# NVlabs/sionna

Measured on NVIDIA H100. Metric: coded bits/s, LDPC5G n=8448 k=4224 BP-20 decode, higher is better.
Workload: dtype f32

## Files before the change

include/sionna_b200.h:

```cpp
#ifndef SIONNA_B200_H
#define SIONNA_B200_H
#include <stddef.h>
#include <stdint.h>

#ifdef __cplusplus
extern "C" {
#endif

#define SB_OK 0
#define SB_EINVAL (-1)
#define SB_ECUDA (-2)
#define SB_ENOMEM (-3)
#define SB_EUNSUPPORTED (-4)

const char* sb_last_error(void);
int sb_device_info(int* sm_count, int* cc_major, int* cc_minor, int* smem_optin_bytes);
int sb_version(void);
int64_t sb_launch_count(void);

typedef struct sb_ldpc_graph sb_ldpc_graph;

enum { SB_CN_BOXPLUS_PHI = 0, SB_CN_BOXPLUS = 1, SB_CN_MINSUM = 2, SB_CN_OFFSET_MINSUM = 3, SB_CN_IDENTITY = 4 };
enum { SB_VN_SUM = 0, SB_VN_IDENTITY = 1 };

int sb_ldpc_graph_create(sb_ldpc_graph** out, int32_t num_cn, int32_t num_vn, int32_t num_edges,
                         const int32_t* h_cn_of_edge, const int32_t* h_vn_of_edge,
                         const int32_t* h_in_map, int32_t n_in,
                         const int32_t* h_out_vn, int32_t n_out,
                         const int32_t* h_schedule, int32_t n_sub, int32_t n_active);
int sb_ldpc_graph_create_ordered(sb_ldpc_graph** out, int32_t num_cn, int32_t num_vn, int32_t num_edges,
                                 const int32_t* h_cn_of_edge, const int32_t* h_vn_of_edge,
                                 const int32_t* h_in_map, int32_t n_in,
                                 const int32_t* h_out_vn, int32_t n_out,
                                 const int32_t* h_schedule, int32_t n_sub, int32_t n_active,
                                 const int32_t* h_cn_view);
void sb_ldpc_graph_destroy(sb_ldpc_graph* g);
int sb_ldpc_graph_set_qc(sb_ldpc_graph* g, int32_t Z, int32_t n_entries, const int32_t* h_base_row,
                         const int32_t* h_base_col, const int32_t* h_shift);
int sb_ldpc_graph_is_qc(const sb_ldpc_graph* g);
int sb_debug_phi(const float* d_x, float* d_scalar, float* d_packed, int64_t n, void* stream);
int sb_ldpc_graph_on_chip(const sb_ldpc_graph* g);
size_t sb_ldpc_workspace_bytes(const sb_ldpc_graph* g);
int sb_ldpc_graph_export(const sb_ldpc_graph* g, int32_t* dims, int32_t* cn_order, int32_t* vn_order,
                         int32_t* slot_of_edge, int32_t* vn_slot, int32_t* cn_off, int32_t* vn_off);

int sb_ldpc_decode(const sb_ldpc_graph* g, const float* d_llr, int64_t batch, int32_t num_iter,
                   int32_t cn_rule, int32_t vn_rule, float offset, float llr_max, int32_t hard_out,
                   const float* d_state_in, float* d_state_out, float* d_out,
                   void* d_workspace, size_t workspace_bytes, void* stream);

int sb_ldpc_decode_early(const sb_ldpc_graph* g, const float* d_llr, int64_t batch, int32_t max_iter, int32_t cn_rule,
                         float offset, float llr_max, int32_t hard_out, float* d_out, int32_t* d_num_iter, void* stream);

int sb_ldpc_flat_init(const float* d_x, const int32_t* d_vn_of_edge, const float* d_state_in, float* d_llr, float* d_v2c,
                      int64_t batch, int32_t num_vn, int32_t num_edges, void* stream);
int sb_ldpc_flat_cn(const float* d_v2c, float* d_c2v, const int32_t* d_cn_ptr, const int32_t* d_v2c_perm,
                    const int32_t* d_cn_list, int32_t num_nodes, int64_t batch, int32_t cn_rule, float offset,
                    float llr_max, void* stream);
int sb_ldpc_flat_vn(const float* d_c2v, const float* d_llr, const int32_t* d_vn_ptr, const int32_t* d_c2v_perm,
                    float* d_v2c, float* d_xhat, int32_t num_vn, int64_t batch, int32_t vn_rule, float llr_max,
                    void* stream);
int sb_ldpc_flat_out(const float* d_xhat, const int32_t* d_out_vn, float* d_out, const float* d_v2c, float* d_state_out,
                     int64_t batch, int32_t n_out, int32_t num_edges, int32_t hard_out, void* stream);

typedef struct sb_ldpc5g_encoder sb_ldpc5g_encoder;
int sb_ldpc5g_encoder_create(sb_ldpc5g_encoder** out, int32_t k, int32_t n, int32_t k_ldpc, int32_t n_ldpc,
                             int32_t g_rows, const int32_t* h_a_ptr, const int32_t* h_a_idx,
                             const int32_t* h_binv_ptr, const int32_t* h_binv_idx, const int32_t* h_c1_ptr,
                             const int32_t* h_c1_idx, const int32_t* h_c2_ptr, const int32_t* h_c2_idx,
                             const int32_t* h_tx_vn);
void sb_ldpc5g_encoder_destroy(sb_ldpc5g_encoder* e);
int sb_ldpc5g_encode(const sb_ldpc5g_encoder* e, const float* d_u, int64_t batch, float* d_c, void* stream);

int sb_binary_source(float* d_out, int64_t n, uint64_t seed, uint64_t offset, void* stream);
int sb_normal(float* d_out, int64_t n, float mean, float stddev, uint64_t seed, uint64_t offset, void* stream);
int sb_uniform(float* d_out, int64_t n, float lo, float hi, uint64_t seed, uint64_t offset, void* stream);
int sb_qam_map(const float* d_bits, const float* d_points, int32_t m, float* d_out, int32_t* d_idx_out,
               int64_t n_sym, void* stream);
int sb_demap(const float* d_y, const float* d_no, int64_t no_inner, const float* d_points, int32_t m, int32_t method,
             const float* d_prior, int64_t prior_inner, float* d_llr, int64_t n_sym, int32_t hard_out, void* stream);
int sb_demap_qam(const float* d_y, const float* d_no, int64_t no_inner, const float* d_levels_re,
                 const float* d_levels_im, int32_t m, int32_t method, float* d_llr, int64_t n_sym, int32_t hard_out,
                 void* stream);
int sb_symbol_demap(const float* d_y, const float* d_no, int64_t no_inner, const float* d_points, int32_t num_points,
                    const float* d_prior, int64_t prior_inner, void* d_out, int64_t n_sym, int32_t hard_out,
                    void* stream);
int sb_awgn(const float* d_x, const float* d_no, int64_t no_inner, float* d_y, int64_t n, uint64_t seed,
            uint64_t offset, void* stream);
int sb_count_errors(const float* d_b, const float* d_b_hat, int64_t rows, int32_t k, int64_t* d_counters, void* stream);

int sb_crc_encode(const float* d_bits, const uint32_t* d_gen_rows, int32_t k, int32_t crc_length, float* d_out,
                  int64_t rows, void* stream);
// ... 170 lines not shown
```

sionna_b200/_lib.py:

```python
import ctypes as C
import os

_HERE = os.path.dirname(os.path.abspath(__file__))
LIB_PATH = os.environ.get("SIONNA_B200_LIB") or os.path.join(_HERE, "libsionna_b200.so")
_lib = None

i32, i64, u64, f32, vp, sz = C.c_int32, C.c_int64, C.c_uint64, C.c_float, C.c_void_p, C.c_size_t
P_i32 = C.POINTER(C.c_int32)

SIGNATURES = {
    "sb_last_error": (C.c_char_p, []),
    "sb_device_info": (i32, [P_i32, P_i32, P_i32, P_i32]),
    "sb_version": (i32, []),
    "sb_launch_count": (i64, []),
    "sb_ldpc_graph_create": (i32, [C.POINTER(vp), i32, i32, i32, vp, vp, vp, i32, vp, i32, vp, i32, i32]),
    "sb_ldpc_graph_create_ordered": (i32, [C.POINTER(vp), i32, i32, i32, vp, vp, vp, i32, vp, i32, vp, i32, i32, vp]),
    "sb_ldpc_graph_destroy": (None, [vp]),
    "sb_ldpc_graph_set_qc": (i32, [vp, i32, i32, vp, vp, vp]),
    "sb_ldpc_graph_is_qc": (i32, [vp]),
    "sb_debug_phi": (i32, [vp, vp, vp, i64, vp]),
    "sb_ldpc_graph_on_chip": (i32, [vp]),
    "sb_ldpc_workspace_bytes": (sz, [vp]),
    "sb_ldpc_decode": (i32, [vp, vp, i64, i32, i32, i32, f32, f32, i32, vp, vp, vp, vp, sz, vp]),
    "sb_ldpc_decode_early": (i32, [vp, vp, i64, i32, i32, f32, f32, i32, vp, vp, vp]),
    "sb_ldpc_flat_init": (i32, [vp, vp, vp, vp, vp, i64, i32, i32, vp]),
    "sb_ldpc_flat_cn": (i32, [vp, vp, vp, vp, vp, i32, i64, i32, f32, f32, vp]),
    "sb_ldpc_flat_vn": (i32, [vp, vp, vp, vp, vp, vp, i32, i64, i32, f32, vp]),
    "sb_ldpc_flat_out": (i32, [vp, vp, vp, vp, vp, i64, i32, i32, i32, vp]),
    "sb_ldpc_graph_export": (i32, [vp, vp, vp, vp, vp, vp, vp, vp]),
    "sb_ldpc5g_encoder_create": (i32, [C.POINTER(vp), i32, i32, i32, i32, i32] + [vp] * 9),
    "sb_ldpc5g_encoder_destroy": (None, [vp]),
    "sb_ldpc5g_encode": (i32, [vp, vp, i64, vp, vp]),
    "sb_binary_source": (i32, [vp, i64, u64, u64, vp]),
    "sb_normal": (i32, [vp, i64, f32, f32, u64, u64, vp]),
    "sb_qam_map": (i32, [vp, vp, i32, vp, vp, i64, vp]),
    "sb_demap": (i32, [vp, vp, i64, vp, i32, i32, vp, i64, vp, i64, i32, vp]),
    "sb_demap_qam": (i32, [vp, vp, i64, vp, vp, i32, i32, vp, i64, i32, vp]),
    "sb_symbol_demap": (i32, [vp, vp, i64, vp, i32, vp, i64, vp, i64, i32, vp]),
    "sb_awgn": (i32, [vp, vp, i64, vp, i64, u64, u64, vp]),
    "sb_count_errors": (i32, [vp, vp, i64, i32, vp, vp]),
    "sb_crc_encode": (i32, [vp, vp, i32, i32, vp, i64, vp]),
    "sb_crc_check": (i32, [vp, vp, i32, i32, vp, vp, i64, vp]),
    "sb_scramble": (i32, [vp, vp, i32, vp, i64, i32, i32, vp]),
    "sb_ofdm_modulate": (i32, [vp, vp, i64, i32, i32, vp, vp, i32, i32, vp]),
    "sb_ofdm_demodulate": (i32, [vp, vp, i64, i32, i32, vp, vp, i32, i32, i32, vp]),
    "sb_gather_rows": (i32, [vp, vp, vp, i64, i32, i32, i32, i32, i32, vp]),
    "sb_rg_map": (i32, [vp, vp, vp, vp, i64, i32, i32, i32, i32, vp]),
    "sb_ls_at_pilots": (i32, [vp, vp, vp, vp, i64, vp, vp, i64, i32, i32, i32, vp]),
    "sb_interp_lin": (i32, [vp] * 8 + [i32, vp, i64, i32, i32, i32, i32, i32, vp]),
    "sb_apply_ofdm_channel": (i32, [vp, vp, vp, i64, vp, i64, i32, i32, i32, i32, u64, u64, vp]),
    "sb_apply_time_channel": (i32, [vp, vp, vp, i64, vp, i64, i32, i32, i32, i32, i32, u64, u64, vp]),
    "sb_uniform": (i32, [vp, i64, f32, f32, u64, u64, vp]),
    "sb_tdl_sos": (i32, [vp, vp, vp, vp, vp, f32, f32, vp, i64, i32, i32, i32, i32, f32, vp]),
    "sb_cdl_coefficients": (i32, [vp] * 15 + [f32, f32, vp, i64, i32, i32, i32, i32, f32, vp]),
    "sb_phase_table": (i32, [vp, vp, f32, i32, vp, i64, i32, i32, vp]),
    "sb_cir_gram": (i32, [vp, vp, i64, i32, i32, vp]),
    "sb_cir_link_scale": (i32, [vp, vp, i64, vp, i64, i32, i32, i32, i32, i32, i32, f32, vp]),
    "sb_cir_apply": (i32, [vp, vp, i64, vp, vp, i64, i32, i32, i32, i32, i32, i32, i32, vp]),
    "sb_spatial_corr": (i32, [vp, vp, vp, i64, i32, i64, vp]),
    "sb_flat_fading": (i32, [vp, i64, u64, u64, vp, i64, vp, i64, i32, vp, vp, i64, vp, i64, u64, u64, vp, i64, i32, i32, vp]),
    "sb_chol_lower": (i32, [vp, vp, i64, i32, vp]),
    "sb_pusch_precode": (i32, [vp, vp, vp, i64, i32, i32, i32, i64, vp]),
    "sb_pusch_ls_combine": (i32, [vp, vp, i64, i32, i32, i32, i32, vp]),
    "sb_lmmse_equalize": (i32, [vp, vp, vp, vp, vp, i64, i32, i32, vp]),
    "sb_mimo_linalg": (i32, [i32, vp, vp, vp, vp, vp, i64, i32, i32, vp]),
    "sb_ofdm_frontend": (i32, [vp] * 15 + [i64] + [i32] * 11 + [vp]),
    "sb_ofdm_lmmse": (i32, [vp] * 12 + [i64] + [i32] * 8 + [vp]),
    "sb_ofdm_equalize": (i32, [i32] + [vp] * 12 + [i64] + [i32] * 8 + [vp]),
    "sb_mimo_ml": (i32, [vp] * 7 + [sz, i64] + [i32] * 6 + [vp]),
    "sb_ml_workspace_bytes": (sz, [i64, i32]),
    "sb_ofdm_ml": (i32, [vp] * 14 + [sz, i64] + [i32] * 12 + [vp]),
    "sb_mimo_kbest": (i32, [vp] * 6 + [sz, i64] + [i32] * 7 + [f32, vp]),
# ... 89 lines not shown
```

sionna_b200/csrc/ldpc_bp_qc.cu:

```cuda
#include <algorithm>
#include <climits>
#include <iterator>
#include <numeric>
#include <vector>
#include "sb_common.h"
#include "sb_math.h"
#include "sb_math2.cuh"
#include "ldpc_graph.h"
#include "ldpc_rules.cuh"

namespace {

constexpr int kLoop = INT_MAX;
constexpr int kRowMax[] = {kLoop, 20, 12, 8, 4};
constexpr int kColCut = 7, kColFused = 10;
constexpr int kColMax[] = {kLoop, 32, 20, 12, 8, 4, 2, kLoop, 12, 4, 1};
constexpr int kRowClasses = (int)std::size(kRowMax);
constexpr int kColClasses = (int)std::size(kColMax);

constexpr bool decreasing(const int* m, int lo, int hi) {
    for (int k = lo + 1; k < hi; ++k)
        if (m[k] >= m[k - 1]) return false;
    return true;
}
static_assert(decreasing(kRowMax, 0, kRowClasses), "row class bounds must decrease");
static_assert(decreasing(kColMax, 0, kColCut) && decreasing(kColMax, kColCut, kColFused), "column class bounds must decrease");
static_assert(kColFused == kColClasses - 1 && kColMax[kColFused] == 1, "the fused class holds degree-1 columns only");

constexpr int degree_class(const int* m, int lo, int hi, int d) {
    int k = hi - 1;
    while (k > lo && d > m[k]) --k;
    return k;
}

struct QcParams {
    int Z, n_rows, n_cols, nnz, N, E, E_alloc, n_in, n_out;
    int row_cls_end[kRowClasses];
    int col_cls_end[kColClasses];
    int row_cls_mod[kRowClasses];
    int col_cls_mod[kColClasses];
    const int4* row_info;
    const int4* col_info;
    const int2* col_edge;
    const int* in_idx;
    const int* out_pos;
    const int* slot_of_edge;
    const float* llr;
    float* out;
    float* state_out;
    long long B;
    int num_iter, hard_out, use_tma;
    int early;
    int* iters_out;
    const int2* row_edge;
    int tab_rep;
    float offset, llr_max;
};


#define SB_PHI_HI 16.635532f
#define SB_PHI_ZERO 14.7117348f
template <class LT, class Probe>
__device__ __forceinline__ uint2 phi_pass1_pair(unsigned b0, unsigned b1, float& P, const LT& lt, Probe probe) {
    const float a0 = __uint_as_float(b0 & 0x7fffffffu), a1 = __uint_as_float(b1 & 0x7fffffffu);
    const float2 p = sb_phif2(make_float2(a0, a1), lt);
    probe(a0, a1);
    P = __fadd_rn(P, p.x);
    P = __fadd_rn(P, p.y);
    return make_uint2(__float_as_uint(p.x) | (b0 & 0x80000000u), __float_as_uint(p.y) | (b1 & 0x80000000u));
}
template <class LT>
__device__ __forceinline__ unsigned phi_pass1(unsigned b0, float& P, const LT& lt) {
    const float p = sb_phif_s(__uint_as_float(b0 & 0x7fffffffu), lt);
    P = __fadd_rn(P, p);
    return __float_as_uint(p) | (b0 & 0x80000000u);
}
template <class LT>
__device__ __forceinline__ uint2 phi_pass2_pair(unsigned w0, unsigned w1, float P, unsigned par, float clip, const LT& lt) {
    const float2 m = fadd2(make_float2(__uint_as_float(w0 | 0x80000000u), __uint_as_float(w1 | 0x80000000u)),
                           make_float2(P, P));
    const float2 y = sb_phif2(m, lt);
    return make_uint2(__float_as_uint(fminf(y.x, clip)) | ((w0 ^ par) & 0x80000000u),
                      __float_as_uint(fminf(y.y, clip)) | ((w1 ^ par) & 0x80000000u));
}
template <class LT>
__device__ __forceinline__ unsigned phi_pass2(unsigned w0, float P, unsigned par, float clip, const LT& lt) {
    const float y = sb_phif_s(__fadd_rn(__uint_as_float(w0 | 0x80000000u), P), lt);
    return __float_as_uint(fminf(y, clip)) | ((w0 ^ par) & 0x80000000u);
}
__device__ __forceinline__ unsigned ldw(const float* q) { return __float_as_uint(*q); }
__device__ __forceinline__ void stw(float* q, unsigned w) { *q = __uint_as_float(w); }

template <class LT>
__device__ __noinline__ void cn_phi_qc(float* pm, int Z, int deg, float clip, int* sat_flag, LT lt) {
    const unsigned am = __activemask();
    float P = 0.f;
    unsigned par = 0;
    int l = 0;
#pragma unroll 2
    for (; l + 1 < deg; l += 2) {
        float* q0 = pm + l * Z;
        float* q1 = q0 + Z;
        const unsigned b0 = ldw(q0), b1 = ldw(q1);
        par ^= b0 ^ b1;
        const uint2 w = phi_pass1_pair(b0, b1, P, lt, [&](float a0, float a1) {
            if (l == 0 && __all_sync(am, a0 >= SB_PHI_HI && a1 >= SB_PHI_HI)) *sat_flag = 1;
        });
        stw(q0, w.x);
        stw(q1, w.y);
// ... 206 lines not shown
    uint32_t j4, j4w, jk;
};
__device__ __forceinline__ uint32_t vn_addr(int2 e, const VnLane& v) {
    return (uint32_t)e.x + (v.jk < (uint32_t)e.y ? v.j4w : v.j4);
}
__device__ __forceinline__ bool vn_in_row(int2 e, uint32_t addr, const VnLane& v) {
    return addr - (uint32_t)e.x - ((uint32_t)e.y >> 16) < ((uint32_t)e.y & 0xffffu);
}

template <int DMAX, bool CHECK, bool KEEPM, bool EXACT = false>
__device__ __forceinline__ float vn_qc(uint32_t ce_s, int deg, const VnLane& vl, float llr, float clip) {
    uint32_t addr[DMAX];
    float m[KEEPM ? DMAX : 1];
    bool on[DMAX];
    float acc = 0.f;
#pragma unroll
    for (int k = 0; k < DMAX; ++k) {
        int2 e = make_int2(0, 0);
        if (EXACT || k < deg) e = lds_i2(ce_s + 8 * k);
        addr[k] = vn_addr(e, vl);
        bool ok = EXACT || ((k < deg) && (!CHECK || vn_in_row(e, addr[k], vl)));
        on[k] = ok;
        float v = 0.f;
        if (ok) v = lds_f32(addr[k]);
        if (ok) acc = __fadd_rn(acc, v);
        if (KEEPM) m[KEEPM ? k : 0] = v;
    }
    float x_tot = __fadd_rn(acc, llr);
#pragma unroll
    for (int k = 0; k < DMAX; ++k) {
        float v = 0.f;
        if (KEEPM) v = m[KEEPM ? k : 0];
        else if (on[k]) v = lds_f32(addr[k]);
        float y = clipf(__fadd_rn(-v, x_tot), clip);
        if (on[k]) sts_f32(addr[k], y);
    }
    return x_tot;
}

template <int MODE>
__device__ __forceinline__ float vn_qc_loop(uint32_t ce_s, int deg, const VnLane& vl, float llr, float clip) {
    float acc = 0.f;
    if (MODE == 0)
        for (int k = 0; k < deg; ++k) {
            const int2 e = lds_i2(ce_s + 8 * k);
            const uint32_t a = vn_addr(e, vl);
            if (vn_in_row(e, a, vl)) acc = __fadd_rn(acc, lds_f32(a));
        }
    float x_tot = __fadd_rn(acc, llr);
    for (int k = 0; k < deg; ++k) {
        const int2 e = lds_i2(ce_s + 8 * k);
        const uint32_t a = vn_addr(e, vl);
        if (vn_in_row(e, a, vl))
            sts_f32(a, (MODE == 1) ? __fadd_rn(llr, 0.f) : clipf(__fadd_rn(-lds_f32(a), x_tot), clip));
    }
    return x_tot;
}

template <int CLS, bool EX>
__device__ __forceinline__ float vn_cls(uint32_t ce, int deg, const VnLane& vl, float llr, float clip) {
    constexpr int D = kColMax[CLS];
    if constexpr (D == kLoop) {
        return vn_qc_loop<0>(ce, deg, vl, llr, clip);
    } else if constexpr (CLS >= kColCut) {
        return vn_qc<D, true, true>(ce, deg, vl, llr, clip);
    } else if constexpr (D > 12) {
        if (CLS == 2 && EX && deg == 19) return vn_qc<19, false, true, true>(ce, deg, vl, llr, clip);
        if (CLS == 2 && EX && deg == 17) return vn_qc<17, false, true, true>(ce, deg, vl, llr, clip);
        return vn_qc<D, false, false>(ce, deg, vl, llr, clip);
    } else {
        if constexpr (CLS == 3) {
            if (EX && deg == 9) return vn_qc<9, false, true, true>(ce, deg, vl, llr, clip);
            if (EX && deg == 10) return vn_qc<10, false, true, true>(ce, deg, vl, llr, clip);
            if (EX && deg == 11) return vn_qc<11, false, true, true>(ce, deg, vl, llr, clip);
        } else if constexpr (CLS == 4) {
            if (EX && deg == 5) return vn_qc<5, false, true, true>(ce, deg, vl, llr, clip);
            if (EX && deg == 6) return vn_qc<6, false, true, true>(ce, deg, vl, llr, clip);
            if (EX && deg == 7) return vn_qc<7, false, true, true>(ce, deg, vl, llr, clip);
        } else if constexpr (CLS == 5) {
            if (EX && deg == 3) return vn_qc<3, false, true, true>(ce, deg, vl, llr, clip);
        } else {
            if (EX && deg == 1) return vn_qc<1, false, true, true>(ce, deg, vl, llr, clip);
        }
        return vn_qc<D, false, true, EX>(ce, deg, vl, llr, clip);
    }
}

struct WarpCtx {
    int G, grp, lane_i;
};

__device__ __forceinline__ int first_of(int start, int start_mod, const WarpCtx& w) {
    return start + (w.grp - start_mod + (w.grp < start_mod ? w.G : 0));
}

__device__ __forceinline__ void fused_vn(const QcParams& p, float* q, float c2v, int fw, int lane_i, const float* llr_s,
                                         float clip, unsigned char* hd) {
    int s = fw >> 16, vb = fw & 0xffff;
    int j = lane_i + s;
    j -= (j >= p.Z) ? p.Z : 0;
    float x_tot = __fadd_rn(__fadd_rn(0.f, c2v), llr_s[vb * p.Z + j]);
    *q = clipf(__fadd_rn(-c2v, x_tot), clip);
    if (hd) hd[vb * p.Z + j] = 0.f >= x_tot ? 1 : 0;
}

template <int RULE, int CLS, class LT>
__device__ __forceinline__ void cn_class(const QcParams& p, const WarpCtx& w, float* msg, const float* llr_s,
// ... 104 lines not shown
        const int4 ri = s_row[rr];
        if (w.lane_i < ri.z) {
            unsigned par = 0;
            for (int l = 0; l < ri.y; ++l) {
                const int2 e = __ldg(p.row_edge + ri.x + l);
                int j = w.lane_i + e.y;
                j -= (j >= p.Z) ? p.Z : 0;
                par ^= hd[e.x + j];
            }
            if (par) *unsat = 1;
        }
    }
}

template <int CLS, bool EX>
__device__ __forceinline__ void vn_class(const QcParams& p, const WarpCtx& w, const VnLane& vl, const float* llr_s,
                                         const int4* s_col, uint32_t s_ce, int start, int end, float clip,
                                         bool final_pass, long long b, unsigned char* hd) {
    for (int cc = first_of(start, p.col_cls_mod[CLS], w); cc < end; cc += w.G) {
        int4 ci = s_col[cc];
        if (w.lane_i < ci.z) {
            int v = ci.w + w.lane_i;
            float x_tot = vn_cls<CLS, EX>(s_ce + 8 * ci.x, ci.y, vl, llr_s[v], clip);
            if (hd) hd[v] = 0.f >= x_tot ? 1 : 0;
            if (final_pass) {
                int o = p.out_pos[v];
                if (o >= 0) {
                    x_tot = clipf(x_tot, clip);
                    p.out[(size_t)b * p.n_out + o] = decoder_out(x_tot, p.hard_out);
                }
            }
        }
    }
}

template <bool EX>
__device__ __forceinline__ void vn_all(const QcParams& p, const WarpCtx& w, const VnLane& vl, const float* llr_s,
                                       const int4* s_col, uint32_t s_ce, float clip, bool final_pass,
                                       bool with_fused, long long b, unsigned char* hd) {
    const int* ce = p.col_cls_end;
    vn_class<0, EX>(p, w, vl, llr_s, s_col, s_ce, 0, ce[0], clip, final_pass, b, hd);
    vn_class<1, EX>(p, w, vl, llr_s, s_col, s_ce, ce[0], ce[1], clip, final_pass, b, hd);
    vn_class<2, EX>(p, w, vl, llr_s, s_col, s_ce, ce[1], ce[2], clip, final_pass, b, hd);
    vn_class<3, EX>(p, w, vl, llr_s, s_col, s_ce, ce[2], ce[3], clip, final_pass, b, hd);
    vn_class<4, EX>(p, w, vl, llr_s, s_col, s_ce, ce[3], ce[4], clip, final_pass, b, hd);
    vn_class<5, EX>(p, w, vl, llr_s, s_col, s_ce, ce[4], ce[5], clip, final_pass, b, hd);
    vn_class<6, EX>(p, w, vl, llr_s, s_col, s_ce, ce[5], ce[6], clip, final_pass, b, hd);
    vn_class<7, EX>(p, w, vl, llr_s, s_col, s_ce, ce[6], ce[7], clip, final_pass, b, hd);
    vn_class<8, EX>(p, w, vl, llr_s, s_col, s_ce, ce[7], ce[8], clip, final_pass, b, hd);
    vn_class<9, EX>(p, w, vl, llr_s, s_col, s_ce, ce[8], ce[9], clip, final_pass, b, hd);
    if (with_fused) vn_class<10, EX>(p, w, vl, llr_s, s_col, s_ce, ce[9], ce[10], clip, final_pass, b, hd);
}

__device__ __forceinline__ void vn_init(const QcParams& p, const WarpCtx& w, const VnLane& vl, const float* llr_s,
                                        const int4* s_col, uint32_t s_ce) {
    for (int cc = w.grp; cc < p.n_cols; cc += w.G) {
        const int4 ci = s_col[cc];
        if (w.lane_i < ci.z) vn_qc_loop<1>(s_ce + 8 * ci.x, ci.y, vl, llr_s[ci.w + w.lane_i], 0.f);
    }
}

constexpr int kQcThreads = 768;

template <int RULE, int REP, bool EARLY>
__global__ void __launch_bounds__(kQcThreads, 1) ldpc_bp_qc_kernel(const __grid_constant__ QcParams p) {
    const int T = blockDim.x, tid = threadIdx.x, lane = tid & 31, warp = tid >> 5, W = T >> 5;
    const int Z = p.Z, N = p.N, Zb = (Z + 31) >> 5;
    unsigned char* const smem_raw = sb_smem + (RULE == SB_CN_BOXPLUS_PHI ? LogTab<REP>::bytes : 0);
    const int off_llr = p.E_alloc * 4;
    const int off_col = (off_llr + N * 4 + 15) & ~15;
    const int off_row = off_col + p.n_cols * 16;
    const int off_ce = off_row + p.n_rows * 16;
    const int off_bar = (off_ce + p.nnz * 8 + 15) & ~15;
    float* msg = reinterpret_cast<float*>(smem_raw);
    float* llr_s = reinterpret_cast<float*>(smem_raw + off_llr);
    int4* s_col = reinterpret_cast<int4*>(smem_raw + off_col);
    int4* s_row = reinterpret_cast<int4*>(smem_raw + off_row);
    int2* s_ce_p = reinterpret_cast<int2*>(smem_raw + off_ce);
    uint64_t* bar = reinterpret_cast<uint64_t*>(smem_raw + off_bar);
    int* sat_flag = reinterpret_cast<int*>(smem_raw + off_bar + 8);
    int* unsat = reinterpret_cast<int*>(smem_raw + off_bar + 12);
    unsigned char* hd = EARLY ? smem_raw + off_bar + 16 : nullptr;
    const uint32_t msgb = smem_u32(smem_raw);
    const uint32_t s_ce = msgb + off_ce;
    WarpCtx w;
    w.G = W / Zb;
    w.grp = warp / Zb;
    w.lane_i = (warp - w.grp * Zb) * 32 + lane;
    VnLane vl{4u * w.lane_i, 4u * (w.lane_i + Z), (4u * w.lane_i) << 16 | 0xffffu};
    asm("" : "+r"(vl.j4), "+r"(vl.j4w), "+r"(vl.jk));

    for (int i = tid; i < p.n_cols; i += T) s_col[i] = p.col_info[i];
    for (int i = tid; i < p.n_rows; i += T) s_row[i] = p.row_info[i];
    for (int i = tid; i < p.nnz; i += T) {
        const int2 e = p.col_edge[i];
        const uint32_t s4 = (uint32_t)e.y & 0xffffu;
        s_ce_p[i] = make_int2((int)(msgb + (uint32_t)e.x - s4), (int)(s4 << 16 | (uint32_t)e.y >> 16));
    }
    const LogTab<REP> lt(lane);
    if (RULE == SB_CN_BOXPLUS_PHI) LogTab<REP>::fill(tid, T);
    if (p.use_tma && tid == 0) mbar_init(bar);
    __syncthreads();

    const float clip = p.llr_max;
    const float phi_max = sb_phif(0.f);
    uint32_t tma_phase = 0;

    for (long long b = blockIdx.x; b < p.B; b += gridDim.x) {
        load_channel_llr(llr_s, p.llr + (size_t)b * p.n_in, p.in_idx, N, p.n_in, clip, p.use_tma, msg, bar, tma_phase,
                         tid, T);
        __syncthreads();
        if (tid == 0) *sat_flag = 0;
        vn_init(p, w, vl, llr_s, s_col, s_ce);
        __syncthreads();
        if (p.num_iter == 0) {
            for (int v = tid; v < N; v += T) {
                int o = p.out_pos[v];
                if (o >= 0) p.out[(size_t)b * p.n_out + o] = decoder_out(llr_s[v], p.hard_out);
            }
        }
        int limit = p.num_iter;
        for (int it = 0; it < limit; ++it) {
            if (EARLY && it > 0 && it < limit - 1) {
                if (tid == 0) *unsat = 0;
                __syncthreads();
                syndrome_pass(p, w, s_row, hd, unsat);
                __syncthreads();
                if (*unsat == 0) limit = it + 1;
            }
            const bool final_pass = it == limit - 1;
            const bool sc = *sat_flag != 0;
            if (final_pass && tid == 0 && p.use_tma && b + gridDim.x < p.B)
                asm volatile("cp.async.bulk.prefetch.L2.global [%0], %1;" ::"l"(p.llr + (size_t)(b + gridDim.x) * p.n_in),
                             "r"((uint32_t)p.n_in * 4u) : "memory");
            if constexpr (RULE == SB_CN_BOXPLUS_PHI) {
                if (sc) cn_vote_pass(p, w, msg, llr_s, s_row, clip, !final_pass, phi_max, sat_flag, lt, hd);
                else cn_all<RULE>(p, w, msg, llr_s, s_row, clip, !final_pass, sat_flag, lt, hd);
            } else {
                cn_all<RULE>(p, w, msg, llr_s, s_row, clip, !final_pass, sat_flag, lt, hd);
            }
            __syncthreads();
            vn_all<true>(p, w, vl, llr_s, s_col, s_ce, clip, final_pass, final_pass, b, hd);
            __syncthreads();
        }
        if (EARLY && p.iters_out && tid == 0) p.iters_out[b] = limit;
        if (p.state_out) {
            store_state(p.state_out + (size_t)b * p.E, msg, p.slot_of_edge, p.E, tid, T);
            __syncthreads();
        }
    }
}

size_t qc_smem_bytes(const sb_ldpc_graph* g, int tab_rep, int early = 0) {
    return (early ? (size_t)g->N + 16 : 0) + ((size_t)g->qc_nnz * g->qc_Z + g->N) * 4 + 16 + (size_t)g->qc_cols * 16 + (size_t)g->qc_rows * 16 +
           (size_t)g->qc_nnz * 8 + 16 + 16 + (size_t)tab_rep * SB_LOGTAB_N * 8;
}

template <int RULE, bool EARLY>
int launch_qc(const QcParams& p, int num_sms, int threads, size_t smem, cudaStream_t stream) {
    auto kern = ldpc_bp_qc_kernel<RULE, 16, EARLY>;
    if constexpr (RULE == SB_CN_BOXPLUS_PHI) {
        if (p.tab_rep == 8) kern = ldpc_bp_qc_kernel<RULE, 8, EARLY>;
        if (p.tab_rep == 1) kern = ldpc_bp_qc_kernel<RULE, 1, EARLY>;
    }
    return sb_launch_decoder(kern, p, num_sms, threads, smem, LLONG_MAX, stream, "sb_ldpc_decode(qc)");
}

}

extern "C" int sb_ldpc_graph_set_qc(sb_ldpc_graph* g, int32_t Z, int32_t n_entries, const int32_t* base_row,
                                    const int32_t* base_col, const int32_t* shift) {
    SB_CHECK_ARG(g && Z > 0 && Z <= 16383 && n_entries > 0 && base_row && base_col && shift, "sb_ldpc_graph_set_qc: bad arguments");
    SB_CHECK_ARG((int)g->h_cn.size() == g->E, "sb_ldpc_graph_set_qc: handle holds no edge list");
    SB_CHECK_ARG(!g->ref_order, "sb_ldpc_graph_set_qc: the QC kernel sums in ascending neighbour order; graphs created with "
                                "sb_ldpc_graph_create_ordered stay on the generic kernel");
    const int C = g->C, N = g->N, E = g->E;
    const int n_rows = (C + Z - 1) / Z, n_cols = (N + Z - 1) / Z;
    auto zrow = [&](int r) { return std::min(Z, C - r * Z); };
    auto zcol = [&](int c) { return std::min(Z, N - c * Z); };
    struct Ent { int r, c, s; };
    std::vector<Ent> ents;
    for (int k = 0; k < n_entries; ++k) {
        if (base_row[k] < 0 || base_col[k] < 0 || shift[k] < 0) { sb_set_error("sb_ldpc_graph_set_qc: negative entry"); return SB_EINVAL; }
        if (base_row[k] >= n_rows || base_col[k] >= n_cols) continue;
        ents.push_back({base_row[k], base_col[k], shift[k] % Z});
    }
    std::vector<long long> keys(E);
    for (int e = 0; e < E; ++e) keys[e] = ((long long)g->h_cn[e] << 32) | (unsigned)g->h_vn[e];
    std::sort(keys.begin(), keys.end());
    long long total = 0;
    for (const Ent& en : ents)
        for (int i = 0; i < zrow(en.r); ++i) {
            int j = (i + en.s) % Z;
            long long key = ((long long)(en.r * Z + i) << 32) | (unsigned)(en.c * Z + j);
            if (j >= zcol(en.c) || !std::binary_search(keys.begin(), keys.end(), key)) {
// ... 52 lines not shown
                    for (size_t q = r0; q < r1; ++q) slots.push_back(q);
                    std::stable_sort(slots.begin(), slots.end(), [&](size_t a, size_t b) { return load[a % G] < load[b % G]; });
                    for (size_t q : slots) {
                        order[q] = items[next++];
                        load[q % G] += deg[order[q]];
                    }
                }
                pos = end;
            }
        };
        balance(rorder, rdeg, row_class);
        balance(corder, cdeg, col_class);
    }
    std::vector<int> row_cls_end(kRowClasses, 0), col_cls_end(kColClasses, 0);
    for (int r = 0; r < n_rows; ++r) for (int k = row_class(r); k < kRowClasses; ++k) ++row_cls_end[k];
    for (int c = 0; c < n_cols; ++c) for (int k = col_class(c); k < kColClasses; ++k) ++col_cls_end[k];
    std::vector<int> be_of((size_t)n_rows * n_cols, -1);
    std::vector<int> row_info(4 * n_rows), row_edge;
    int be = 0;
    for (int rr = 0; rr < n_rows; ++rr) {
        int r = rorder[rr];
        row_info[4 * rr] = be;
        row_info[4 * rr + 1] = rdeg[r];
        row_info[4 * rr + 2] = zrow(r);
        row_info[4 * rr + 3] = fused_col_of_row[r] >= 0 ? (fused_col_of_row[r] | (by_row[r].back().s << 16)) : -1;
        for (const Ent& en : by_row[r]) {
            if (be_of[(size_t)en.r * n_cols + en.c] != -1) { sb_set_error("sb_ldpc_graph_set_qc: duplicate base entry"); return SB_EINVAL; }
            be_of[(size_t)en.r * n_cols + en.c] = be++;
            row_edge.push_back(en.c * Z);
            row_edge.push_back(en.s);
        }
    }
    const int nnz = be;
    std::vector<int> col_info(4 * n_cols), col_edge(2 * (size_t)nnz);
    int ce = 0;
    for (int cc = 0; cc < n_cols; ++cc) {
        int c = corder[cc];
        col_info[4 * cc] = ce;
        for (const Ent& en : by_col[c]) {
            col_edge[2 * ce] = be_of[(size_t)en.r * n_cols + en.c] * Z * 4;
            col_edge[2 * ce + 1] = (en.s * 4) | ((zrow(en.r) * 4) << 16);
            ++ce;
        }
        col_info[4 * cc + 1] = cdeg[c];
        col_info[4 * cc + 2] = zcol(c);
        col_info[4 * cc + 3] = c * Z;
    }
    std::vector<int> in_nat(N), out_nat(N), slot(E);
    for (int r = 0; r < N; ++r) { in_nat[g->vn_order[r]] = g->in_idx[r]; out_nat[g->vn_order[r]] = g->out_pos[r]; }
    for (int e = 0; e < E; ++e) {
        int r = g->h_cn[e] / Z, i = g->h_cn[e] % Z, c = g->h_vn[e] / Z;
        slot[e] = be_of[(size_t)r * n_cols + c] * Z + i;
    }
    g->qc = true; g->qc_Z = Z; g->qc_rows = n_rows; g->qc_cols = n_cols; g->qc_nnz = nnz;
    g->qc_max_row_deg = *std::max_element(rdeg.begin(), rdeg.end());
    g->qc_max_col_deg = *std::max_element(cdeg.begin(), cdeg.end());
    g->qc_row_info.swap(row_info); g->qc_col_info.swap(col_info); g->qc_col_edge.swap(col_edge);
    g->qc_row_cls_end = row_cls_end; g->qc_col_cls_end = col_cls_end;
    g->qc_in_idx.swap(in_nat); g->qc_out_pos.swap(out_nat); g->qc_slot_of_edge.swap(slot); g->qc_row_edge.swap(row_edge);
    g->qc_tables.set(g->qc_row_info, g->qc_col_info, g->qc_col_edge, g->qc_in_idx, g->qc_out_pos, g->qc_slot_of_edge,
                     g->qc_row_edge);
    return SB_OK;
}

namespace {
__global__ void debug_phi_kernel(const float* x, float* o1, float* o2, long long n) {
    LogTab<16>::fill(threadIdx.x, blockDim.x);
    __syncthreads();
    const LogTab<16> lt(threadIdx.x & 31);
    long long i = (long long)blockIdx.x * blockDim.x + threadIdx.x;
    if (2 * i + 1 < n) {
        float2 r = sb_phif2(make_float2(x[2 * i], x[2 * i + 1]), lt);
        o2[2 * i] = r.x; o2[2 * i + 1] = r.y;
        o1[2 * i] = sb_phif(x[2 * i]); o1[2 * i + 1] = sb_phif(x[2 * i + 1]);
    }
}
}
extern "C" int sb_debug_phi(const float* d_x, float* d_scalar, float* d_packed, int64_t n, void* stream) {
    if (n == 0) return SB_OK;
    SB_CHECK_ARG(d_x && d_scalar && d_packed && n >= 0 && n % 2 == 0, "sb_debug_phi: bad arguments");
    debug_phi_kernel<<<(unsigned)((n / 2 + 255) / 256), 256, LogTab<16>::bytes, (cudaStream_t)stream>>>(d_x, d_scalar,
                                                                                                         d_packed, n);
    SB_LAUNCH_CHECK();
    return SB_OK;
}

extern "C" int sb_ldpc_graph_is_qc(const sb_ldpc_graph* g) { return g && g->qc ? 1 : 0; }

int sb_qc_try_decode(const sb_ldpc_graph* g, const DeviceTables::Copy& dev, const float* d_llr, int64_t batch,
                     int32_t num_iter, int32_t cn_rule, int32_t vn_rule, float offset, float llr_max, int32_t hard_out,
                     const float* d_state_in, float* d_state_out, float* d_out, cudaStream_t stream, bool* handled,
                     int32_t early, int32_t* d_iters) {
    *handled = false;
    if (!g->qc || !g->flooding || vn_rule != SB_VN_SUM || d_state_in || cn_rule > SB_CN_OFFSET_MINSUM) return SB_OK;
    int tab_rep = cn_rule == SB_CN_BOXPLUS_PHI ? 16 : 0;
    if (tab_rep && qc_smem_bytes(g, tab_rep, early) > (size_t)dev.smem_optin) tab_rep = 8;
    if (tab_rep && qc_smem_bytes(g, tab_rep, early) > (size_t)dev.smem_optin) tab_rep = 1;
    const size_t smem = qc_smem_bytes(g, tab_rep, early);
    if (smem > (size_t)dev.smem_optin) return SB_OK;
    if ((cn_rule == SB_CN_MINSUM || cn_rule == SB_CN_OFFSET_MINSUM) &&
        !(llr_max < 100000.f && (float)(g->qc_max_row_deg - 1) * llr_max < 99000.f))
        return SB_OK;
    const DeviceTables::Copy* d = nullptr;
    int rc = g->qc_tables.get(&d);
    if (rc) return rc;
    QcParams p{};
    p.Z = g->qc_Z; p.n_rows = g->qc_rows; p.n_cols = g->qc_cols; p.nnz = g->qc_nnz; p.N = g->N; p.E = g->E;
    p.E_alloc = g->qc_nnz * g->qc_Z; p.n_in = g->n_in; p.n_out = g->n_out;
    for (int k = 0; k < kRowClasses; ++k) p.row_cls_end[k] = g->qc_row_cls_end[k];
    for (int k = 0; k < kColClasses; ++k) p.col_cls_end[k] = g->qc_col_cls_end[k];
    p.row_info = d->at<int4>(0); p.col_info = d->at<int4>(1);
    p.col_edge = d->at<int2>(2); p.in_idx = d->at<int>(3); p.out_pos = d->at<int>(4);
    p.slot_of_edge = d->at<int>(5);
    p.llr = d_llr; p.out = d_out; p.state_out = d_state_out; p.B = batch; p.num_iter = num_iter; p.hard_out = hard_out;
    p.offset = offset; p.llr_max = llr_max; p.tab_rep = tab_rep;
    p.early = early; p.iters_out = d_iters; p.row_edge = d->at<int2>(6);
    p.use_tma = (g->n_in % 4 == 0) && (g->n_in <= p.E_alloc) && ((reinterpret_cast<uintptr_t>(d_llr) & 15) == 0);
    const int Zb = (g->qc_Z + 31) / 32;
    const int max_warps = kQcThreads / 32;
    int groups = std::max(1, std::min(max_warps / Zb, std::max(g->qc_rows, g->qc_cols)));
    const int threads = groups * Zb * 32;
    for (int k = 0; k < kRowClasses; ++k) p.row_cls_mod[k] = (k ? g->qc_row_cls_end[k - 1] : 0) % groups;
    for (int k = 0; k < kColClasses; ++k) p.col_cls_mod[k] = (k ? g->qc_col_cls_end[k - 1] : 0) % groups;
    rc = sb_dispatch<SB_CN_BOXPLUS_PHI, SB_CN_OFFSET_MINSUM>(cn_rule, [&](auto R) {
        return p.early ? launch_qc<R, true>(p, dev.num_sms, threads, smem, stream)
                       : launch_qc<R, false>(p, dev.num_sms, threads, smem, stream);
    });
    *handled = (rc == SB_OK);
    return rc;
}
```

sionna_b200/csrc/ldpc_graph.h:

```cpp
#pragma once
#include <stdint.h>
#include <algorithm>
#include <vector>
#include "sb_common.h"

struct sb_ldpc_graph {
    int C = 0, N = 0, E = 0, Lc = 0, Lv = 0, n_in = 0, n_out = 0, n_sub = 1, n_active = 0;
    bool flooding = true;
    bool ref_order = false;
    std::vector<int> cn_off, cn_cnt, vn_off, vn_cnt, in_idx, out_pos, slot_of_edge, sched, cn_order, vn_order;
    std::vector<uint32_t> vn_slot;
    std::vector<uint16_t> vn_slot16;
    std::vector<int> h_cn, h_vn;
    mutable DeviceTables tables;
    bool qc = false;
    int qc_Z = 0, qc_rows = 0, qc_cols = 0, qc_nnz = 0, qc_max_row_deg = 0, qc_max_col_deg = 0;
    std::vector<int> qc_row_info;
    std::vector<int> qc_col_info;
    std::vector<int> qc_col_edge;
    std::vector<int> qc_in_idx, qc_out_pos, qc_slot_of_edge;
    std::vector<int> qc_row_edge;
    std::vector<int> qc_row_cls_end, qc_col_cls_end;
    mutable DeviceTables qc_tables;
};

static const int kSmemOptinH100 = 232448;

int sb_qc_try_decode(const sb_ldpc_graph* g, const DeviceTables::Copy& dev, const float* d_llr, int64_t batch,
                     int32_t num_iter, int32_t cn_rule, int32_t vn_rule, float offset, float llr_max, int32_t hard_out,
                     const float* d_state_in, float* d_state_out, float* d_out, cudaStream_t stream, bool* handled,
                     int32_t early = 0, int32_t* d_iters = nullptr);

#if defined(__CUDACC__)
template <class Kernel, class Params>
int sb_launch_decoder(Kernel kern, const Params& p, int num_sms, int threads, size_t smem, long long max_grid,
                      cudaStream_t stream, const char* who) {
    SB_CUDA(cudaFuncSetAttribute(kern, cudaFuncAttributeMaxDynamicSharedMemorySize, (int)smem));
    int occ = 0;
    SB_CUDA(cudaOccupancyMaxActiveBlocksPerMultiprocessor(&occ, kern, threads, smem));
    if (occ < 1) { sb_set_error("%s: kernel does not fit (threads %d, smem %zu)", who, threads, smem); return SB_EUNSUPPORTED; }
    long long grid = std::min<long long>(p.B, std::min<long long>((long long)num_sms * occ, max_grid));
    kern<<<(unsigned)grid, threads, smem, stream>>>(p);
    SB_LAUNCH_CHECK();
    return SB_OK;
}

__device__ __forceinline__ float clipf(float x, float c) { return fminf(fmaxf(x, -c), c); }

__device__ __forceinline__ uint32_t smem_u32(const void* p) { return (uint32_t)__cvta_generic_to_shared(p); }
__device__ __forceinline__ void mbar_init(uint64_t* bar) {
    asm volatile("mbarrier.init.shared::cta.b64 [%0], %1;" ::"r"(smem_u32(bar)), "r"(1));
    asm volatile("fence.mbarrier_init.release.cluster;" ::: "memory");
}
__device__ __forceinline__ void mbar_expect_tx(uint64_t* bar, uint32_t bytes) {
    asm volatile("mbarrier.arrive.expect_tx.shared::cta.b64 _, [%0], %1;" ::"r"(smem_u32(bar)), "r"(bytes) : "memory");
}
__device__ __forceinline__ void mbar_wait(uint64_t* bar, uint32_t parity) {
    asm volatile(
        "{\n"
        ".reg .pred p;\n"
        "WAIT_%=:\n"
        "mbarrier.try_wait.parity.shared::cta.b64 p, [%0], %1;\n"
        "@p bra DONE_%=;\n"
        "bra WAIT_%=;\n"
        "DONE_%=:\n"
        "}\n" ::"r"(smem_u32(bar)), "r"(parity) : "memory");
}
__device__ __forceinline__ void tma_bulk_g2s(void* dst_smem, const void* src_gmem, uint32_t bytes, uint64_t* bar) {
    asm volatile("cp.async.bulk.shared::cluster.global.mbarrier::complete_tx::bytes [%0], [%1], %2, [%3];" ::"r"(
                     smem_u32(dst_smem)),
                 "l"(src_gmem), "r"(bytes), "r"(smem_u32(bar))
                 : "memory");
}

__device__ __forceinline__ float decoder_out(float x, int hard_out) {
// ... 34 lines not shown
```

sionna_b200/phy/fec/ldpc/decoding.py:

```python
import os
import types
import numpy as np
import scipy as sp
import scipy.sparse
import torch

from ...block import Block
from ...._lib import Handle, lib, check, ptr, current_stream
from .encoding import LDPC5GEncoder

_CN_RULES = {"boxplus-phi": 0, "boxplus": 1, "minsum": 2, "min": 2, "offset-minsum": 3, "identity": 4}
_VN_RULES = {"sum": 0, "identity": 1}


def _i32(a):
    return np.ascontiguousarray(np.asarray(a), dtype=np.int32)


class _GraphHandle(Handle):

    def __init__(self, num_cn, num_vn, cn_idx, vn_idx, in_map=None, n_in=0, out_vn=None, n_out=0, schedule=None,
                 cn_view=None):
        cn_idx, vn_idx = _i32(cn_idx), _i32(vn_idx)
        in_map = None if in_map is None else _i32(in_map)
        out_vn = None if out_vn is None else _i32(out_vn)
        n_sub = n_active = 0
        if schedule is not None:
            schedule = _i32(schedule)
            n_sub, n_active = schedule.shape
        args = (num_cn, num_vn, len(vn_idx), ptr(cn_idx), ptr(vn_idx), ptr(in_map), int(n_in), ptr(out_vn), int(n_out),
                ptr(schedule), int(n_sub), int(n_active))
        if cn_view is None:
            super().__init__("ldpc_graph", *args)
        else:
            cn_view = _i32(cn_view)
            super().__init__("ldpc_graph", *args, ptr(cn_view), create="sb_ldpc_graph_create_ordered")
        self.num_edges = len(vn_idx)
        self.n_in = int(n_in) if in_map is not None else num_vn
        self.n_out = int(n_out) if out_vn is not None else num_vn
        self._ws = None

    def on_chip(self):
        return bool(lib().sb_ldpc_graph_on_chip(self.handle))

    def set_qc(self, z, base_row, base_col, shift):
        r, c, s = _i32(base_row), _i32(base_col), _i32(shift)
        return lib().sb_ldpc_graph_set_qc(self.handle, int(z), len(r), ptr(r), ptr(c), ptr(s)) == 0

    def is_qc(self):
        return bool(lib().sb_ldpc_graph_is_qc(self.handle))

    def workspace(self, device):
        need = lib().sb_ldpc_workspace_bytes(self.handle)
        if need == 0:
            return None, 0
        if self._ws is None or self._ws.numel() < need or self._ws.device != device:
            self._ws = torch.empty(need, dtype=torch.uint8, device=device)
        return self._ws, need

    def export(self):
        dims = np.zeros(10, np.int32)
        check(lib().sb_ldpc_graph_export(self.handle, ptr(dims), None, None, None, None, None, None), "export")
        c, n, e, lc, lv = (int(x) for x in dims[:5])
        out = {"dims": dims, "cn_order": np.zeros(c, np.int32), "vn_order": np.zeros(n, np.int32),
               "slot_of_edge": np.zeros(e, np.int32), "vn_slot": np.zeros(e, np.int32),
               "cn_off": np.zeros(lc + 1, np.int32), "vn_off": np.zeros(lv + 1, np.int32)}
        check(lib().sb_ldpc_graph_export(self.handle, ptr(dims), ptr(out["cn_order"]), ptr(out["vn_order"]),
                                         ptr(out["slot_of_edge"]), ptr(out["vn_slot"]), ptr(out["cn_off"]),
                                         ptr(out["vn_off"])), "export")
        return out


class LDPCBPDecoder(Block):

    def __init__(self, pcm, cn_update="boxplus-phi", vn_update="sum", cn_schedule="flooding", hard_out=True,
                 num_iter=20, llr_max=20., v2c_callbacks=None, c2v_callbacks=None, return_state=False,
                 precision=None, **kwargs):
        if "cn_type" in kwargs:
            raise TypeError("'cn_type' is deprecated; use 'cn_update' instead.")
        self._early_stop = bool(kwargs.pop("early_stop", False))
        self.num_iter_run = None
        sum_order = kwargs.pop("sum_order", "ascending")
        if sum_order not in ("ascending", "reference"):
            raise ValueError("sum_order must be 'ascending' or 'reference'.")
        self._sum_order = sum_order
        super().__init__(precision=precision, **kwargs)
        if not isinstance(hard_out, bool):
            raise TypeError("hard_out must be bool.")
        if not isinstance(num_iter, int):
            raise TypeError("num_iter must be int.")
        if num_iter < 0:
            raise ValueError("num_iter cannot be negative.")
        if not isinstance(return_state, bool):
            raise TypeError("return_state must be bool.")
        if isinstance(pcm, np.ndarray):
            if not np.array_equal(pcm, pcm.astype(bool)):
                raise ValueError("PC matrix must be binary.")
        elif isinstance(pcm, (sp.sparse.csr_matrix, sp.sparse.csc_matrix)):
            if not np.array_equal(pcm.data, pcm.data.astype(bool)):
                raise ValueError("PC matrix must be binary.")
        else:
            raise TypeError("Unsupported dtype of pcm.")
        if not isinstance(llr_max, (int, float)):
# ... 371 lines not shown
```

Baseline: 3.096 billion.

## Specialize first two BP iterations for punctured columns in QC decoder

Adds an 'opening' path for the boxplus-phi QC decoder that exploits known structure in the first two iterations. Punctured (zero-LLR) columns are tracked per row as a bitmask, and the variable-node update after iteration 0 is restricted to those columns. The messages are pre-staged in phi-transformed form during init so the first check-node pass can skip work on non-punctured edges. The goal is to cut arithmetic in the early iterations, at the cost of extra code paths, extra table lookups and possible register pressure or divergence.

```diff
diff --git a/include/sionna_b200.h b/include/sionna_b200.h
--- a/include/sionna_b200.h
+++ b/include/sionna_b200.h
@@ -38,6 +38,7 @@
 int sb_ldpc_graph_set_qc(sb_ldpc_graph* g, int32_t Z, int32_t n_entries, const int32_t* h_base_row,
                          const int32_t* h_base_col, const int32_t* h_shift);
 int sb_ldpc_graph_is_qc(const sb_ldpc_graph* g);
+int sb_ldpc_graph_qc_opening(const sb_ldpc_graph* g);
 int sb_debug_phi(const float* d_x, float* d_scalar, float* d_packed, int64_t n, void* stream);
 int sb_ldpc_graph_on_chip(const sb_ldpc_graph* g);
 size_t sb_ldpc_workspace_bytes(const sb_ldpc_graph* g);
diff --git a/sionna_b200/_lib.py b/sionna_b200/_lib.py
--- a/sionna_b200/_lib.py
+++ b/sionna_b200/_lib.py
@@ -18,6 +18,7 @@
     "sb_ldpc_graph_destroy": (None, [vp]),
     "sb_ldpc_graph_set_qc": (i32, [vp, i32, i32, vp, vp, vp]),
     "sb_ldpc_graph_is_qc": (i32, [vp]),
+    "sb_ldpc_graph_qc_opening": (i32, [vp]),
     "sb_debug_phi": (i32, [vp, vp, vp, i64, vp]),
     "sb_ldpc_graph_on_chip": (i32, [vp]),
     "sb_ldpc_workspace_bytes": (sz, [vp]),
diff --git a/sionna_b200/csrc/ldpc_bp_qc.cu b/sionna_b200/csrc/ldpc_bp_qc.cu
--- a/sionna_b200/csrc/ldpc_bp_qc.cu
+++ b/sionna_b200/csrc/ldpc_bp_qc.cu
@@ -55,6 +55,8 @@
     const int2* row_edge;
     int tab_rep;
     float offset, llr_max;
+    int open;
+    const int* open_tab;
 };
 
 
@@ -367,7 +369,7 @@
         const int2 e = lds_i2(ce_s + 8 * k);
         const uint32_t a = vn_addr(e, vl);
         if (vn_in_row(e, a, vl))
-            sts_f32(a, (MODE == 1) ? __fadd_rn(llr, 0.f) : clipf(__fadd_rn(-lds_f32(a), x_tot), clip));
+            sts_f32(a, (MODE == 1) ? __fadd_rn(llr, 0.f) : (MODE == 2) ? llr : clipf(__fadd_rn(-lds_f32(a), x_tot), clip));
     }
     return x_tot;
 }
@@ -578,11 +580,103 @@
     if (with_fused) vn_class<10, EX>(p, w, vl, llr_s, s_col, s_ce, ce[9], ce[10], clip, final_pass, b, hd);
 }
 
+template <class LT>
 __device__ __forceinline__ void vn_init(const QcParams& p, const WarpCtx& w, const VnLane& vl, const float* llr_s,
-                                        const int4* s_col, uint32_t s_ce) {
+                                        const int4* s_col, uint32_t s_ce, bool staged, const LT& lt) {
     for (int cc = w.grp; cc < p.n_cols; cc += w.G) {
         const int4 ci = s_col[cc];
-        if (w.lane_i < ci.z) vn_qc_loop<1>(s_ce + 8 * ci.x, ci.y, vl, llr_s[ci.w + w.lane_i], 0.f);
+        if (w.lane_i >= ci.z) continue;
+        const float llr = llr_s[ci.w + w.lane_i];
+        if (staged) {
+            float P = 0.f;
+            const unsigned st = phi_pass1(__float_as_uint(__fadd_rn(llr, 0.f)), P, lt);
+            vn_qc_loop<2>(s_ce + 8 * ci.x, ci.y, vl, __uint_as_float(st), 0.f);
+        } else {
+            vn_qc_loop<1>(s_ce + 8 * ci.x, ci.y, vl, llr, 0.f);
+        }
+    }
+}
+
+template <class LT>
+__device__ __noinline__ void cn_phi_open(float* pm, int Z, int deg, unsigned punct, bool second, float clip, LT lt) {
+    float P = 0.f;
+    unsigned u = second ? punct : 0u;
+    for (; u & (u - 1); u &= u - 1) {
+        float* q0 = pm + (__ffs(u) - 1) * Z;
+        u &= u - 1;
+        float* q1 = pm + (__ffs(u) - 1) * Z;
+        const uint2 w = phi_pass1_pair(ldw(q0), ldw(q1), P, lt, [](float, float) {});
+        stw(q0, w.x);
+        stw(q1, w.y);
+    }
+    if (u) {
+        float* q0 = pm + (__ffs(u) - 1) * Z;
+        stw(q0, phi_pass1(ldw(q0), P, lt));
+    }
+    P = 0.f;
+    unsigned par = 0;
+    for (int l = 0; l < deg; ++l) {
+        const unsigned w = ldw(pm + l * Z);
+        par ^= w;
+        P = __fadd_rn(P, __uint_as_float(w & 0x7fffffffu));
+    }
+    par &= 0x80000000u;
+    if (!second && (punct & (punct - 1))) {
+        for (u = punct; u; u &= u - 1) {
+            float* q0 = pm + (__ffs(u) - 1) * Z;
+            stw(q0, (ldw(q0) ^ par) & 0x80000000u);
+        }
+        return;
+    }
+    for (u = second ? 0xffffffffu >> (32 - deg) : punct; u & (u - 1); u &= u - 1) {
+        float* q0 = pm + (__ffs(u) - 1) * Z;
+        u &= u - 1;
+        float* q1 = pm + (__ffs(u) - 1) * Z;
+        const uint2 y = phi_pass2_pair(ldw(q0), ldw(q1), P, par, clip, lt);
+        stw(q0, y.x);
+        stw(q1, y.y);
+    }
+    if (u) {
+        float* q0 = pm + (__ffs(u) - 1) * Z;
+        stw(q0, phi_pass2(ldw(q0), P, par, clip, lt));
+    }
+}
+
+template <class LT>
+__device__ __forceinline__ void cn_open_pass(const QcParams& p, const WarpCtx& w, float* msg, const float* llr_s,
+                                             const int4* s_row, float clip, bool second, int* sat_flag, const LT& lt) {
+    const int Z = p.Z;
+    for (int rr = w.grp; rr < p.n_rows; rr += w.G) {
+        const int4 ri = s_row[rr];
+        if (w.lane_i < ri.z) {
+            const unsigned punct = (unsigned)__ldg(p.open_tab + rr);
+            float* pm = msg + ri.x * Z + w.lane_i;
+            if (second && ri.y >= 2) {
+                auto mag = [&](int l) {
+                    if ((punct >> l) & 1u) return fabsf(pm[l * Z]);
+                    const int2 e = __ldg(p.row_edge + ri.x + l);
+                    int j = w.lane_i + e.y;
+                    j -= (j >= Z) ? Z : 0;
+                    return fabsf(llr_s[e.x + j]);
+                };
+                const float a0 = mag(0), a1 = mag(1);
+                if (__all_sync(__activemask(), a0 >= SB_PHI_HI && a1 >= SB_PHI_HI)) *sat_flag = 1;
+            }
+            cn_phi_open<LT>(pm, Z, ri.y, punct, second, clip, lt);
+            if (second && ri.w >= 0) {
+                float* q = pm + (ri.y - 1) * Z;
+                fused_vn(p, q, *q, ri.w, w.lane_i, llr_s, clip, nullptr);
+            }
+        }
+    }
+}
+
+__device__ __forceinline__ void vn_open(const QcParams& p, const WarpCtx& w, const VnLane& vl, const float* llr_s,
+                                        const int4* s_col, uint32_t s_ce, float clip) {
+    for (int cc = w.grp; cc < p.n_cols; cc += w.G) {
+        const int4 ci = s_col[cc];
+        if (__ldg(p.open_tab + p.n_rows + cc) && w.lane_i < ci.z)
+            vn_qc_loop<0>(s_ce + 8 * ci.x, ci.y, vl, llr_s[ci.w + w.lane_i], clip);
     }
 }
 
@@ -631,13 +725,14 @@
     const float clip = p.llr_max;
     const float phi_max = sb_phif(0.f);
     uint32_t tma_phase = 0;
+    const bool open = RULE == SB_CN_BOXPLUS_PHI && !EARLY && p.open && p.num_iter >= 3;
 
     for (long long b = blockIdx.x; b < p.B; b += gridDim.x) {
         load_channel_llr(llr_s, p.llr + (size_t)b * p.n_in, p.in_idx, N, p.n_in, clip, p.use_tma, msg, bar, tma_phase,
                          tid, T);
         __syncthreads();
         if (tid == 0) *sat_flag = 0;
-        vn_init(p, w, vl, llr_s, s_col, s_ce);
+        vn_init(p, w, vl, llr_s, s_col, s_ce, open, lt);
         __syncthreads();
         if (p.num_iter == 0) {
             for (int v = tid; v < N; v += T) {
@@ -660,13 +755,15 @@
                 asm volatile("cp.async.bulk.prefetch.L2.global [%0], %1;" ::"l"(p.llr + (size_t)(b + gridDim.x) * p.n_in),
                              "r"((uint32_t)p.n_in * 4u) : "memory");
             if constexpr (RULE == SB_CN_BOXPLUS_PHI) {
-                if (sc) cn_vote_pass(p, w, msg, llr_s, s_row, clip, !final_pass, phi_max, sat_flag, lt, hd);
+                if (open && it < 2) cn_open_pass(p, w, msg, llr_s, s_row, clip, it == 1, sat_flag, lt);
+                else if (sc) cn_vote_pass(p, w, msg, llr_s, s_row, clip, !final_pass, phi_max, sat_flag, lt, hd);
                 else cn_all<RULE>(p, w, msg, llr_s, s_row, clip, !final_pass, sat_flag, lt, hd);
             } else {
                 cn_all<RULE>(p, w, msg, llr_s, s_row, clip, !final_pass, sat_flag, lt, hd);
             }
             __syncthreads();
-            vn_all<true>(p, w, vl, llr_s, s_col, s_ce, clip, final_pass, final_pass, b, hd);
+            if (open && it == 0) vn_open(p, w, vl, llr_s, s_col, s_ce, clip);
+            else vn_all<true>(p, w, vl, llr_s, s_col, s_ce, clip, final_pass, final_pass, b, hd);
             __syncthreads();
         }
         if (EARLY && p.iters_out && tid == 0) p.iters_out[b] = limit;
@@ -825,14 +922,32 @@
         int r = g->h_cn[e] / Z, i = g->h_cn[e] % Z, c = g->h_vn[e] / Z;
         slot[e] = be_of[(size_t)r * n_cols + c] * Z + i;
     }
-    g->qc = true; g->qc_Z = Z; g->qc_rows = n_rows; g->qc_cols = n_cols; g->qc_nnz = nnz;
+    std::vector<int> open_tab(n_rows + n_cols, 0);
+    bool open = true;
+    std::vector<char> punct(n_cols, 1);
+    for (int c = 0; c < n_cols; ++c)
+        for (int v = c * Z; v < c * Z + zcol(c); ++v) punct[c] = punct[c] && in_nat[v] == -1;
+    for (int rr = 0; rr < n_rows; ++rr) {
+        const int r = rorder[rr];
+        unsigned m = 0;
+        for (size_t l = 0; l < by_row[r].size() && l < 32; ++l) m |= (unsigned)punct[by_row[r][l].c] << l;
+        open = open && rdeg[r] <= 32 && (m & 3u);
+        open_tab[rr] = (int)m;
+    }
+    for (int cc = 0; cc < n_cols; ++cc) {
+        open_tab[n_rows + cc] = punct[corder[cc]];
+        open = open && !(punct[corder[cc]] && col_fused[corder[cc]]);
+    }
+    g->qc = true;
+    g->qc_open = open;
+    g->qc_open_tab.swap(open_tab); g->qc_Z = Z; g->qc_rows = n_rows; g->qc_cols = n_cols; g->qc_nnz = nnz;
     g->qc_max_row_deg = *std::max_element(rdeg.begin(), rdeg.end());
     g->qc_max_col_deg = *std::max_element(cdeg.begin(), cdeg.end());
     g->qc_row_info.swap(row_info); g->qc_col_info.swap(col_info); g->qc_col_edge.swap(col_edge);
     g->qc_row_cls_end = row_cls_end; g->qc_col_cls_end = col_cls_end;
     g->qc_in_idx.swap(in_nat); g->qc_out_pos.swap(out_nat); g->qc_slot_of_edge.swap(slot); g->qc_row_edge.swap(row_edge);
     g->qc_tables.set(g->qc_row_info, g->qc_col_info, g->qc_col_edge, g->qc_in_idx, g->qc_out_pos, g->qc_slot_of_edge,
-                     g->qc_row_edge);
+                     g->qc_row_edge, g->qc_open_tab);
     return SB_OK;
 }
 
@@ -859,6 +974,7 @@
 }
 
 extern "C" int sb_ldpc_graph_is_qc(const sb_ldpc_graph* g) { return g && g->qc ? 1 : 0; }
+extern "C" int sb_ldpc_graph_qc_opening(const sb_ldpc_graph* g) { return g && g->qc && g->qc_open ? 1 : 0; }
 
 int sb_qc_try_decode(const sb_ldpc_graph* g, const DeviceTables::Copy& dev, const float* d_llr, int64_t batch,
                      int32_t num_iter, int32_t cn_rule, int32_t vn_rule, float offset, float llr_max, int32_t hard_out,
@@ -888,6 +1004,8 @@
     p.llr = d_llr; p.out = d_out; p.state_out = d_state_out; p.B = batch; p.num_iter = num_iter; p.hard_out = hard_out;
     p.offset = offset; p.llr_max = llr_max; p.tab_rep = tab_rep;
     p.early = early; p.iters_out = d_iters; p.row_edge = d->at<int2>(6);
+    p.open = cn_rule == SB_CN_BOXPLUS_PHI && g->qc_open && llr_max >= 0.f;
+    p.open_tab = d->at<int>(7);
     p.use_tma = (g->n_in % 4 == 0) && (g->n_in <= p.E_alloc) && ((reinterpret_cast<uintptr_t>(d_llr) & 15) == 0);
     const int Zb = (g->qc_Z + 31) / 32;
     const int max_warps = kQcThreads / 32;
diff --git a/sionna_b200/csrc/ldpc_graph.h b/sionna_b200/csrc/ldpc_graph.h
--- a/sionna_b200/csrc/ldpc_graph.h
+++ b/sionna_b200/csrc/ldpc_graph.h
@@ -21,6 +21,8 @@
     std::vector<int> qc_in_idx, qc_out_pos, qc_slot_of_edge;
     std::vector<int> qc_row_edge;
     std::vector<int> qc_row_cls_end, qc_col_cls_end;
+    bool qc_open = false;
+    std::vector<int> qc_open_tab;
     mutable DeviceTables qc_tables;
 };
 
diff --git a/sionna_b200/phy/fec/ldpc/decoding.py b/sionna_b200/phy/fec/ldpc/decoding.py
--- a/sionna_b200/phy/fec/ldpc/decoding.py
+++ b/sionna_b200/phy/fec/ldpc/decoding.py
@@ -49,6 +49,9 @@
 
     def is_qc(self):
         return bool(lib().sb_ldpc_graph_is_qc(self.handle))
+
+    def qc_opening(self):
+        return bool(lib().sb_ldpc_graph_qc_opening(self.handle))
 
     def workspace(self, device):
         need = lib().sb_ldpc_workspace_bytes(self.handle)
```

After: 3.228 billion, median of 6. 1.04x the previous value.
